# MCG-NJU/MeMOTR

Hardware: AMD Instinct MI355X
Metric: train_frames_per_sec (higher is better)
Workload: dtype f32

## Files before the change

memotr_amd/csrc/clip_ops.hip:

```cpp
#include <hip/hip_runtime.h>
#include <stdint.h>
#include <stdio.h>

#include <atomic>

#include "../../include/clip_ops_hip.h"
#include "assign_core.h"

namespace {

thread_local char g_err[256] = {0};

int fail(int code, const char *msg) {
    snprintf(g_err, sizeof(g_err), "%s", msg);
    return code;
}

int check_launch(const char *what) {
    const hipError_t e = hipGetLastError();
    if (e != hipSuccess) {
        snprintf(g_err, sizeof(g_err), "%s: %s", what, hipGetErrorString(e));
        return (int)e;
    }
    g_err[0] = 0;
// ... 371 lines not shown
    if ((threadIdx.x & 63) == 0) s_w[threadIdx.x >> 6] = a;
    __syncthreads();
    if (threadIdx.x == 0) {
        const f64x4_t t = (s_w[0] + s_w[1]) + (s_w[2] + s_w[3]);
        const f32x4_t r = {(float)t.x, (float)t.y, (float)t.z, (float)t.w};
        *reinterpret_cast<f32x4_t *>(out + c) = r;
    }
}

__device__ __forceinline__ float colsum_ld(const float *x, long i) { return x[i]; }
__device__ __forceinline__ float colsum_ld(const uint16_t *x, long i) {
    return __uint_as_float(((unsigned)x[i]) << 16);
}

template <typename TX>
__global__ __launch_bounds__(256) void colsum_partial_kernel(const TX *__restrict__ x, long rows, int cols,
                                                            int chunk_rows, float *__restrict__ partial) {
    __shared__ double s_part[8][33];
    const int tx = threadIdx.x & 31, ty = threadIdx.x >> 5;
    const int c = blockIdx.x * 32 + tx;
    const long r0 = (long)blockIdx.y * chunk_rows;
    const long r1 = r0 + chunk_rows < rows ? r0 + chunk_rows : rows;
    double a0 = 0., a1 = 0., a2 = 0., a3 = 0.;
    if (c < cols) {
        long r = r0 + ty;
        for (; r + 24 < r1; r += 32) {
            a0 += colsum_ld(x, r * cols + c);
            a1 += colsum_ld(x, (r + 8) * cols + c);
            a2 += colsum_ld(x, (r + 16) * cols + c);
            a3 += colsum_ld(x, (r + 24) * cols + c);
        }
        for (; r < r1; r += 8) a0 += colsum_ld(x, r * cols + c);
    }
    s_part[ty][tx] = (a0 + a1) + (a2 + a3);
    __syncthreads();
    if (ty == 0 && c < cols) {
        double t = s_part[0][tx];
#pragma unroll
        for (int i = 1; i < 8; ++i) t += s_part[i][tx];
        partial[(long)blockIdx.y * cols + c] = (float)t;
    }
}

__device__ __forceinline__ void colsum_st(float *x, long i, float v) { x[i] = v; }

template <typename TX>
__global__ __launch_bounds__(256) void relu_bwd_colsum_partial_kernel(const TX *__restrict__ g, const TX *__restrict__ y,
                                                                     long rows, int cols, int chunk_rows,
                                                                     TX *__restrict__ g2, float *__restrict__ partial) {
    __shared__ double s_part[8][33];
    const int tx = threadIdx.x & 31, ty = threadIdx.x >> 5;
    const int c = blockIdx.x * 32 + tx;
    const long r0 = (long)blockIdx.y * chunk_rows;
    const long r1 = r0 + chunk_rows < rows ? r0 + chunk_rows : rows;
    double a0 = 0., a1 = 0., a2 = 0., a3 = 0.;
    if (c < cols) {
        long r = r0 + ty;
        for (; r + 24 < r1; r += 32) {
            const long i0 = r * cols + c, i1 = (r + 8) * cols + c, i2 = (r + 16) * cols + c, i3 = (r + 24) * cols + c;
            const float v0 = colsum_ld(y, i0) <= 0.f ? 0.f : colsum_ld(g, i0);
            const float v1 = colsum_ld(y, i1) <= 0.f ? 0.f : colsum_ld(g, i1);
            const float v2 = colsum_ld(y, i2) <= 0.f ? 0.f : colsum_ld(g, i2);
            const float v3 = colsum_ld(y, i3) <= 0.f ? 0.f : colsum_ld(g, i3);
            colsum_st(g2, i0, v0); colsum_st(g2, i1, v1); colsum_st(g2, i2, v2); colsum_st(g2, i3, v3);
            a0 += v0; a1 += v1; a2 += v2; a3 += v3;
        }
        for (; r < r1; r += 8) {
            const long i0 = r * cols + c;
            const float v0 = colsum_ld(y, i0) <= 0.f ? 0.f : colsum_ld(g, i0);
            colsum_st(g2, i0, v0);
            a0 += v0;
        }
    }
    s_part[ty][tx] = (a0 + a1) + (a2 + a3);
    __syncthreads();
    if (ty == 0 && c < cols) {
        double t = s_part[0][tx];
#pragma unroll
        for (int i = 1; i < 8; ++i) t += s_part[i][tx];
        partial[(long)blockIdx.y * cols + c] = (float)t;
    }
}

constexpr int kLanes = 16;
constexpr int kRows = 256 / kLanes;
constexpr int kHd = 32;
constexpr int kPitch = 36;

__device__ __forceinline__ void load_row32(const float *p, float *r) {
#pragma unroll
    for (int i = 0; i < 8; ++i) {
        const f32x4_t v = *reinterpret_cast<const f32x4_t *>(p + 4 * i);
        r[4 * i] = v.x; r[4 * i + 1] = v.y; r[4 * i + 2] = v.z; r[4 * i + 3] = v.w;
    }
}

__device__ __forceinline__ float dot32(const float *a, const float *lds_row) {
    float s0 = 0.f, s1 = 0.f;
#pragma unroll
    for (int i = 0; i < 8; ++i) {
        const f32x4_t v = *reinterpret_cast<const f32x4_t *>(lds_row + 4 * i);
        s0 = fmaf(a[4 * i], v.x, s0);
        s1 = fmaf(a[4 * i + 1], v.y, s1);
        s0 = fmaf(a[4 * i + 2], v.z, s0);
        s1 = fmaf(a[4 * i + 3], v.w, s1);
    }
    return s0 + s1;
}

__device__ __forceinline__ float dot32r(const float *a, const float *b) {
    float s0 = 0.f, s1 = 0.f;
#pragma unroll
    for (int i = 0; i < 8; ++i) {
        s0 = fmaf(a[4 * i], b[4 * i], s0);
        s1 = fmaf(a[4 * i + 1], b[4 * i + 1], s1);
        s0 = fmaf(a[4 * i + 2], b[4 * i + 2], s0);
        s1 = fmaf(a[4 * i + 3], b[4 * i + 3], s1);
    }
    return s0 + s1;
}

__device__ __forceinline__ void axpy32(float *acc, float w, const float *lds_row) {
#pragma unroll
    for (int i = 0; i < 8; ++i) {
        const f32x4_t v = *reinterpret_cast<const f32x4_t *>(lds_row + 4 * i);
        acc[4 * i] = fmaf(w, v.x, acc[4 * i]);
        acc[4 * i + 1] = fmaf(w, v.y, acc[4 * i + 1]);
        acc[4 * i + 2] = fmaf(w, v.z, acc[4 * i + 2]);
        acc[4 * i + 3] = fmaf(w, v.w, acc[4 * i + 3]);
    }
}

__device__ __forceinline__ float sum8l(float x) {
#pragma unroll
    for (int o = 1; o < kLanes; o <<= 1) x += __shfl_xor(x, o, 64);
    return x;
}
__device__ __forceinline__ float max8l(float x) {
#pragma unroll
    for (int o = 1; o < kLanes; o <<= 1) x = fmaxf(x, __shfl_xor(x, o, 64));
    return x;
}

__device__ __forceinline__ void stage_rows(float *dst, const float *src, long rs, int L) {
    for (int i = threadIdx.x; i < L * 8; i += blockDim.x) {
        const int r = i >> 3, c = (i & 7) * 4;
        *reinterpret_cast<f32x4_t *>(dst + r * kPitch + c) = *reinterpret_cast<const f32x4_t *>(src + r * rs + c);
    }
}

__global__ __launch_bounds__(256) void mha_fwd_kernel(const float *__restrict__ q, const float *__restrict__ k,
                                                     const float *__restrict__ v, long q_bs, long q_rs, long k_bs,
                                                     long k_rs, long v_bs, long v_rs,
                                                     const uint8_t *__restrict__ key_mask, int H, int L, float scale,
                                                     float *__restrict__ out, float *__restrict__ lse) {
    extern __shared__ __attribute__((aligned(16))) float s_mem[];
    float *Ks = s_mem, *Vs = s_mem + (size_t)L * kPitch;
    const int h = blockIdx.y, b = blockIdx.z;
    stage_rows(Ks, k + b * k_bs + h * kHd, k_rs, L);
    stage_rows(Vs, v + b * v_bs + h * kHd, v_rs, L);
    __syncthreads();
    const int row = blockIdx.x * kRows + threadIdx.x / kLanes, sub = threadIdx.x % kLanes;
    const bool row_ok = row < L;
    const int rowc = row_ok ? row : L - 1;
    float qr[kHd];
    load_row32(q + b * q_bs + rowc * q_rs + h * kHd, qr);
#pragma unroll
    for (int i = 0; i < kHd; ++i) qr[i] *= scale;
    const uint8_t *mk = key_mask ? key_mask + (long)b * L : nullptr;
    float m = -INFINITY, l = 0.f, acc[kHd];
#pragma unroll
    for (int i = 0; i < kHd; ++i) acc[i] = 0.f;
    for (int j = sub; j < L; j += kLanes) {
        if (mk && mk[j]) continue;
        const float s = dot32(qr, Ks + j * kPitch);
        const float m_new = fmaxf(m, s);
        const float corr = expf(m - m_new), p = expf(s - m_new);
        l = l * corr + p;
#pragma unroll
        for (int i = 0; i < kHd; ++i) acc[i] *= corr;
        axpy32(acc, p, Vs + j * kPitch);
        m = m_new;
    }
    const float M = max8l(m);
    const float w = (m == -INFINITY) ? 0.f : expf(m - M);
    const float Lsum = sum8l(l * w);
    const float inv = 1.f / Lsum;
    float *o = out + ((long)b * L + rowc) * (H * kHd) + h * kHd;
#pragma unroll
    for (int i = 0; i < kHd; ++i) {
        const float t = sum8l(acc[i] * w) * inv;
        if (row_ok && (i >> 2) == sub) o[i] = t;
    }
    if (row_ok && sub == 0) lse[((long)b * H + h) * L + row] = M + logf(Lsum);
}

__global__ __launch_bounds__(256) void mha_bwd_q_kernel(const float *__restrict__ q, const float *__restrict__ k,
                                                       const float *__restrict__ v, long q_bs, long q_rs, long k_bs,
                                                       long k_rs, long v_bs, long v_rs,
                                                       const uint8_t *__restrict__ key_mask,
                                                       const float *__restrict__ out, const float *__restrict__ lse,
                                                       const float *__restrict__ go, int H, int L, float scale,
                                                       float *__restrict__ gq, long gq_bs, long gq_rs) {
    extern __shared__ __attribute__((aligned(16))) float s_mem[];
    float *Ks = s_mem, *Vs = s_mem + (size_t)L * kPitch;
    const int h = blockIdx.y, b = blockIdx.z;
    stage_rows(Ks, k + b * k_bs + h * kHd, k_rs, L);
    stage_rows(Vs, v + b * v_bs + h * kHd, v_rs, L);
    __syncthreads();
    const int row = blockIdx.x * kRows + threadIdx.x / kLanes, sub = threadIdx.x % kLanes;
    const bool row_ok = row < L;
    const int rowc = row_ok ? row : L - 1;
    float qr[kHd], gr[kHd], acc[kHd];
    load_row32(q + b * q_bs + rowc * q_rs + h * kHd, qr);
    const long orow = ((long)b * L + rowc) * (H * kHd) + h * kHd;
    load_row32(go + orow, gr);
    float D = 0.f;
    {
        float orr[kHd];
        load_row32(out + orow, orr);
        D = dot32r(gr, orr);
    }
#pragma unroll
    for (int i = 0; i < kHd; ++i) { qr[i] *= scale; acc[i] = 0.f; }
    const float ls = lse[((long)b * H + h) * L + rowc];
    const uint8_t *mk = key_mask ? key_mask + (long)b * L : nullptr;
    for (int j = sub; j < L; j += kLanes) {
        if (mk && mk[j]) continue;
        const float p = expf(dot32(qr, Ks + j * kPitch) - ls);
        const float ds = p * (dot32(gr, Vs + j * kPitch) - D);
        axpy32(acc, ds, Ks + j * kPitch);
    }
    float *g = gq + b * gq_bs + rowc * gq_rs + h * kHd;
#pragma unroll
    for (int i = 0; i < kHd; ++i) {
        const float t = sum8l(acc[i]) * scale;
        if (row_ok && (i >> 2) == sub) g[i] = t;
    }
}

__global__ __launch_bounds__(256) void mha_bwd_kv_kernel(const float *__restrict__ q, const float *__restrict__ k,
                                                        const float *__restrict__ v, long q_bs, long q_rs, long k_bs,
                                                        long k_rs, long v_bs, long v_rs,
                                                        const uint8_t *__restrict__ key_mask,
                                                        const float *__restrict__ out, const float *__restrict__ lse,
                                                        const float *__restrict__ go, int H, int L, float scale,
                                                        float *__restrict__ gk, long gk_bs, long gk_rs,
                                                        float *__restrict__ gv, long gv_bs, long gv_rs) {
    extern __shared__ __attribute__((aligned(16))) float s_mem[];
    float *Qs = s_mem, *Gs = s_mem + (size_t)L * kPitch;
    float *s_lse = Gs + (size_t)L * kPitch, *s_D = s_lse + L;
    const int h = blockIdx.y, b = blockIdx.z;
    stage_rows(Qs, q + b * q_bs + h * kHd, q_rs, L);
    for (int i = threadIdx.x; i < L * 8; i += blockDim.x) {
        f32x4_t *p4 = reinterpret_cast<f32x4_t *>(Qs + (i >> 3) * kPitch + (i & 7) * 4);
        *p4 = *p4 * scale;
    }
    stage_rows(Gs, go + (long)b * L * (H * kHd) + h * kHd, (long)H * kHd, L);
    for (int i = threadIdx.x; i < L; i += blockDim.x) s_lse[i] = lse[((long)b * H + h) * L + i];
    __syncthreads();
    for (int i = threadIdx.x; i < L; i += blockDim.x) {
        const float *o = out + ((long)b * L + i) * (H * kHd) + h * kHd;
        float orr[kHd];
        load_row32(o, orr);
        s_D[i] = dot32(orr, Gs + i * kPitch);
    }
    __syncthreads();
    const int row = blockIdx.x * kRows + threadIdx.x / kLanes, sub = threadIdx.x % kLanes;
    const bool row_ok = row < L;
    const int rowc = row_ok ? row : L - 1;
    const bool dead = key_mask && key_mask[(long)b * L + rowc];
    float kr[kHd], vr[kHd], ak[kHd], av[kHd];
    load_row32(k + b * k_bs + rowc * k_rs + h * kHd, kr);
    load_row32(v + b * v_bs + rowc * v_rs + h * kHd, vr);
#pragma unroll
    for (int i = 0; i < kHd; ++i) { ak[i] = 0.f; av[i] = 0.f; }
    if (!dead) {
        for (int i = sub; i < L; i += kLanes) {
            const float p = expf(dot32(kr, Qs + i * kPitch) - s_lse[i]);
            const float ds = p * (dot32(vr, Gs + i * kPitch) - s_D[i]);
            axpy32(av, p, Gs + i * kPitch);
            axpy32(ak, ds, Qs + i * kPitch);
        }
    }
    float *pk = gk + b * gk_bs + rowc * gk_rs + h * kHd, *pv = gv + b * gv_bs + rowc * gv_rs + h * kHd;
#pragma unroll
    for (int i = 0; i < kHd; ++i) {
        const float tk = sum8l(ak[i]), tv = sum8l(av[i]);
        if (row_ok && (i >> 2) == sub) {
            pk[i] = tk;
            pv[i] = tv;
        }
    }
}

int allow_lds(const void *kernel, size_t lds, std::atomic<unsigned long long> &done) {
    if (lds <= 64 * 1024) return 0;
    int dev = 0;
    (void)hipGetDevice(&dev);
    const unsigned long long bit = 1ull << (dev & 63);
    if (done.load(std::memory_order_acquire) & bit) return 0;
    const hipError_t e = hipFuncSetAttribute(kernel, hipFuncAttributeMaxDynamicSharedMemorySize, 160 * 1024 - 2048);
    if (e != hipSuccess) {
        snprintf(g_err, sizeof(g_err), "hipFuncSetAttribute: %s", hipGetErrorString(e));
        return (int)e;
    }
    done.fetch_or(bit, std::memory_order_release);
    return 0;
}

std::atomic<unsigned long long> g_lds_fwd{0}, g_lds_bq{0}, g_lds_bkv{0};

int mha_check(const void *q, const void *k, const void *v, int B, int H, int L) {
    if (B < 0 || H <= 0 || L < 0) return fail(1, "clipops_mha: bad dimension");
    if (L > CLIPOPS_MHA_MAX_L) return fail(2, "clipops_mha: L exceeds CLIPOPS_MHA_MAX_L");
    if ((long)B * L > 0 && (!q || !k || !v)) return fail(1, "clipops_mha: null pointer");
    return 0;
}

__device__ __forceinline__ float wave_sum64(float x) {
#pragma unroll
    for (int o = 32; o > 0; o >>= 1) x += __shfl_xor(x, o, 64);
    return x;
}

template <bool WITH_Q>
__global__ __launch_bounds__(256) void add_layer_norm_fwd_kernel(const float *__restrict__ x,
                                                                const float *__restrict__ res,
                                                                const float *__restrict__ gamma,
                                                                const float *__restrict__ beta,
                                                                const float *__restrict__ pos, long rows, float eps,
                                                                float *__restrict__ sum, float *__restrict__ y,
                                                                float *__restrict__ q, float *__restrict__ stats) {
    const int lane = threadIdx.x & 63;
    const long row = (long)blockIdx.x * 4 + (threadIdx.x >> 6);
    if (row >= rows) return;
    const long off = row * CLIPOPS_LN_COLS + lane * 4;
    const f32x4_t a = *reinterpret_cast<const f32x4_t *>(x + off);
    const f32x4_t b = *reinterpret_cast<const f32x4_t *>(res + off);
    const f32x4_t s = a + b;
    *reinterpret_cast<f32x4_t *>(sum + off) = s;
    const float mean = wave_sum64((s.x + s.y) + (s.z + s.w)) * (1.f / CLIPOPS_LN_COLS);
    const f32x4_t d = s - mean;
    const float var = wave_sum64((d.x * d.x + d.y * d.y) + (d.z * d.z + d.w * d.w)) * (1.f / CLIPOPS_LN_COLS);
    const float rstd = rsqrtf(var + eps);
    const f32x4_t g = *reinterpret_cast<const f32x4_t *>(gamma + lane * 4);
    const f32x4_t be = *reinterpret_cast<const f32x4_t *>(beta + lane * 4);
    const f32x4_t yv = (d * rstd) * g + be;
    *reinterpret_cast<f32x4_t *>(y + off) = yv;
    if (WITH_Q) *reinterpret_cast<f32x4_t *>(q + off) = yv + *reinterpret_cast<const f32x4_t *>(pos + off);
    if (lane == 0) {
        stats[2 * row] = mean;
        stats[2 * row + 1] = rstd;
    }
}

__global__ __launch_bounds__(256) void add_layer_norm_bwd_kernel(const float *__restrict__ gy,
                                                                const float *__restrict__ sum,
                                                                const float *__restrict__ stats,
                                                                const float *__restrict__ gamma, long rows,
                                                                int chunk_rows, float *__restrict__ gsum,
                                                                float *__restrict__ partial) {
    __shared__ f32x4_t s_acc[4][2][64];
    const int lane = threadIdx.x & 63, wave = threadIdx.x >> 6;
    const f32x4_t gm = *reinterpret_cast<const f32x4_t *>(gamma + lane * 4);
    f32x4_t acc_g = {0.f, 0.f, 0.f, 0.f}, acc_b = {0.f, 0.f, 0.f, 0.f};
    const long r0 = (long)blockIdx.x * chunk_rows;
    const long r1 = r0 + chunk_rows < rows ? r0 + chunk_rows : rows;
    for (long row = r0 + wave; row < r1; row += 4) {
        const long off = row * CLIPOPS_LN_COLS + lane * 4;
        const f32x4_t g = *reinterpret_cast<const f32x4_t *>(gy + off);
        const f32x4_t s = *reinterpret_cast<const f32x4_t *>(sum + off);
        const float mean = stats[2 * row], rstd = stats[2 * row + 1];
        const f32x4_t xh = (s - mean) * rstd;
        const f32x4_t gh = g * gm;
        const float c1 = wave_sum64((gh.x + gh.y) + (gh.z + gh.w)) * (1.f / CLIPOPS_LN_COLS);
        const float c2 = wave_sum64((gh.x * xh.x + gh.y * xh.y) + (gh.z * xh.z + gh.w * xh.w)) * (1.f / CLIPOPS_LN_COLS);
        *reinterpret_cast<f32x4_t *>(gsum + off) = (gh - c1 - xh * c2) * rstd;
        acc_g += g * xh;
        acc_b += g;
    }
    s_acc[wave][0][lane] = acc_g;
    s_acc[wave][1][lane] = acc_b;
    __syncthreads();
    if (wave < 2) {
        const f32x4_t t = (s_acc[0][wave][lane] + s_acc[1][wave][lane]) + (s_acc[2][wave][lane] + s_acc[3][wave][lane]);
        *reinterpret_cast<f32x4_t *>(partial + (long)blockIdx.x * 2 * CLIPOPS_LN_COLS + wave * CLIPOPS_LN_COLS + lane * 4) = t;
    }
}

__global__ __launch_bounds__(256) void add_layer_norm_bwd_fanin_kernel(const float *__restrict__ ga,
                                                                      const float *__restrict__ gb,
                                                                      const float *__restrict__ gc,
                                                                      const float *__restrict__ sum,
// ... 549 lines not shown
    if (!delta || !ref || !out_head || !out_dec) return fail(1, "clipops_refine_boxes_split_fwd_f32: null pointer");
    if (out_head == out_dec) return fail(1, "clipops_refine_boxes_split_fwd_f32: the two outputs alias");
    const bool vec = (((uintptr_t)delta | (uintptr_t)ref | (uintptr_t)out_head | (uintptr_t)out_dec) & 15) == 0;
    if (vec)
        hipLaunchKernelGGL(refine_boxes_split_fwd_kernel<true>, dim3(grid_for(n_rows)), dim3(256), 0,
                           (hipStream_t)stream, delta, ref, n_rows, eps, out_head, out_dec);
    else
        hipLaunchKernelGGL(refine_boxes_split_fwd_kernel<false>, dim3(grid_for(n_rows)), dim3(256), 0,
                           (hipStream_t)stream, delta, ref, n_rows, eps, out_head, out_dec);
    return check_launch("refine_boxes_split_fwd_kernel");
}

int clipops_refine_boxes_bwd_f32(const float *out, const float *ref, const float *grad_out, long n, float eps,
                                 float *grad_delta, float *grad_ref, void *stream) {
    if (n < 0) return fail(1, "clipops_refine_boxes_bwd_f32: negative count");
    if (n == 0) { g_err[0] = 0; return 0; }
    if (!out || !ref || !grad_out || !grad_delta) return fail(1, "clipops_refine_boxes_bwd_f32: null pointer");
    hipLaunchKernelGGL(refine_boxes_bwd_kernel, dim3(grid_for(n)), dim3(256), 0, (hipStream_t)stream, out, ref,
                       grad_out, n, eps, grad_delta, grad_ref);
    return check_launch("refine_boxes_bwd_kernel");
}

int clipops_colsum_f32(const float *x, long rows, int cols, float *out, void *stream) {
    if (rows < 0 || cols < 0) return fail(1, "clipops_colsum_f32: bad dimension");
    if (cols == 0) { g_err[0] = 0; return 0; }
    if (!out || (rows > 0 && !x)) return fail(1, "clipops_colsum_f32: null pointer");
    if (cols % 4 == 0 && rows <= 2048 && (((uintptr_t)x | (uintptr_t)out) & 15) == 0) {
        hipLaunchKernelGGL(colsum_quad_kernel, dim3(cols / 4), dim3(256), 0, (hipStream_t)stream, x, rows, cols, out);
        return check_launch("colsum_quad_kernel");
    }
    hipLaunchKernelGGL(colsum_kernel, dim3((cols + 31) / 32), dim3(256), 0, (hipStream_t)stream, x, rows, cols, out);
    return check_launch("colsum_kernel");
}

int clipops_colsum_partial_f32(const float *x, long rows, int cols, int chunk_rows, float *partial, void *stream) {
    if (rows < 0 || cols < 0 || chunk_rows <= 0) return fail(1, "clipops_colsum_partial_f32: bad dimension");
    if (cols == 0 || rows == 0) { g_err[0] = 0; return 0; }
    if (!x || !partial) return fail(1, "clipops_colsum_partial_f32: null pointer");
    const long chunks = (rows + chunk_rows - 1) / chunk_rows;
    if (chunks > 65535) return fail(1, "clipops_colsum_partial_f32: too many chunks");
    hipLaunchKernelGGL(colsum_partial_kernel<float>, dim3((cols + 31) / 32, (unsigned)chunks), dim3(256), 0,
                       (hipStream_t)stream, x, rows, cols, chunk_rows, partial);
    return check_launch("colsum_partial_kernel");
}

int clipops_colsum_partial_bf16(const uint16_t *x, long rows, int cols, int chunk_rows, float *partial, void *stream) {
    if (rows < 0 || cols < 0 || chunk_rows <= 0) return fail(1, "clipops_colsum_partial_bf16: bad dimension");
    if (cols == 0 || rows == 0) { g_err[0] = 0; return 0; }
    if (!x || !partial) return fail(1, "clipops_colsum_partial_bf16: null pointer");
    const long chunks = (rows + chunk_rows - 1) / chunk_rows;
    if (chunks > 65535) return fail(1, "clipops_colsum_partial_bf16: too many chunks");
    hipLaunchKernelGGL(colsum_partial_kernel<uint16_t>, dim3((cols + 31) / 32, (unsigned)chunks), dim3(256), 0,
                       (hipStream_t)stream, x, rows, cols, chunk_rows, partial);
    return check_launch("colsum_partial_kernel<bf16>");
}

static int relu_bwd_colsum_check(const void *g, const void *y, const void *g2, const void *partial, long rows, int cols,
                                 int chunk_rows, long *chunks) {
    if (rows < 0 || cols < 0 || chunk_rows <= 0) return fail(1, "clipops_relu_bwd_colsum_partial: bad dimension");
    *chunks = (rows + chunk_rows - 1) / chunk_rows;
    if (cols == 0 || rows == 0) return 0;
    if (!g || !y || !g2 || !partial) return fail(1, "clipops_relu_bwd_colsum_partial: null pointer");
    if (*chunks > 65535) return fail(1, "clipops_relu_bwd_colsum_partial: too many chunks");
    return 0;
}

int clipops_relu_bwd_colsum_partial_f32(const float *g, const float *y, long rows, int cols, int chunk_rows, float *g2,
                                        float *partial, void *stream) {
    long chunks = 0;
    if (relu_bwd_colsum_check(g, y, g2, partial, rows, cols, chunk_rows, &chunks)) return 1;
    if (cols == 0 || rows == 0) { g_err[0] = 0; return 0; }
    hipLaunchKernelGGL(relu_bwd_colsum_partial_kernel<float>, dim3((cols + 31) / 32, (unsigned)chunks), dim3(256), 0,
                       (hipStream_t)stream, g, y, rows, cols, chunk_rows, g2, partial);
    return check_launch("relu_bwd_colsum_partial_kernel");
}

int clipops_mha_fwd_f32(const float *q, const float *k, const float *v, long q_bs, long q_rs, long k_bs, long k_rs,
                        long v_bs, long v_rs, const uint8_t *key_mask, int B, int H, int L, float scale, float *out,
                        float *lse, void *stream) {
    int rc = mha_check(q, k, v, B, H, L);
    if (rc) return rc;
    if ((long)B * L == 0) { g_err[0] = 0; return 0; }
    if (!out || !lse) return fail(1, "clipops_mha_fwd_f32: null pointer");
    const size_t lds = (size_t)2 * L * kPitch * sizeof(float);
    if ((rc = allow_lds(reinterpret_cast<const void *>(mha_fwd_kernel), lds, g_lds_fwd))) return rc;
    hipLaunchKernelGGL(mha_fwd_kernel, dim3((L + kRows - 1) / kRows, H, B), dim3(256), lds, (hipStream_t)stream, q, k, v, q_bs,
                       q_rs, k_bs, k_rs, v_bs, v_rs, key_mask, H, L, scale, out, lse);
    return check_launch("mha_fwd_kernel");
}

int clipops_mha_bwd_f32(const float *q, const float *k, const float *v, long q_bs, long q_rs, long k_bs, long k_rs,
                        long v_bs, long v_rs, const uint8_t *key_mask, const float *out, const float *lse,
                        const float *grad_out, int B, int H, int L, float scale, float *grad_q, long gq_bs, long gq_rs,
                        float *grad_k, long gk_bs, long gk_rs, float *grad_v, long gv_bs, long gv_rs, void *stream) {
    int rc = mha_check(q, k, v, B, H, L);
    if (rc) return rc;
    if ((long)B * L == 0) { g_err[0] = 0; return 0; }
    if (!out || !lse || !grad_out || !grad_q || !grad_k || !grad_v) return fail(1, "clipops_mha_bwd_f32: null pointer");
    const size_t lds_q = (size_t)2 * L * kPitch * sizeof(float);
    const size_t lds_kv = lds_q + (size_t)2 * L * sizeof(float);
    if ((rc = allow_lds(reinterpret_cast<const void *>(mha_bwd_q_kernel), lds_q, g_lds_bq))) return rc;
    if ((rc = allow_lds(reinterpret_cast<const void *>(mha_bwd_kv_kernel), lds_kv, g_lds_bkv))) return rc;
    const dim3 grid((L + kRows - 1) / kRows, H, B);
    hipLaunchKernelGGL(mha_bwd_q_kernel, grid, dim3(256), lds_q, (hipStream_t)stream, q, k, v, q_bs, q_rs, k_bs, k_rs,
                       v_bs, v_rs, key_mask, out, lse, grad_out, H, L, scale, grad_q, gq_bs, gq_rs);
    if ((rc = check_launch("mha_bwd_q_kernel"))) return rc;
    hipLaunchKernelGGL(mha_bwd_kv_kernel, grid, dim3(256), lds_kv, (hipStream_t)stream, q, k, v, q_bs, q_rs, k_bs, k_rs,
                       v_bs, v_rs, key_mask, out, lse, grad_out, H, L, scale, grad_k, gk_bs, gk_rs, grad_v, gv_bs, gv_rs);
    return check_launch("mha_bwd_kv_kernel");
}

int clipops_add_layer_norm_fwd_f32(const float *x, const float *res, const float *gamma, const float *beta, long rows,
                                   float eps, float *sum, float *y, float *stats, void *stream) {
    if (rows < 0) return fail(1, "clipops_add_layer_norm_fwd_f32: negative row count");
    if (rows == 0) { g_err[0] = 0; return 0; }
    if (!x || !res || !gamma || !beta || !sum || !y || !stats) return fail(1, "clipops_add_layer_norm_fwd_f32: null pointer");
    hipLaunchKernelGGL(add_layer_norm_fwd_kernel<false>, dim3((unsigned)((rows + 3) / 4)), dim3(256), 0, (hipStream_t)stream,
                       x, res, gamma, beta, nullptr, rows, eps, sum, y, nullptr, stats);
    return check_launch("add_layer_norm_fwd_kernel");
}

int clipops_add_layer_norm_pos_fwd_f32(const float *x, const float *res, const float *gamma, const float *beta,
                                       const float *pos, long rows, float eps, float *sum, float *y, float *q,
                                       float *stats, void *stream) {
    if (rows < 0) return fail(1, "clipops_add_layer_norm_pos_fwd_f32: negative row count");
    if (rows == 0) { g_err[0] = 0; return 0; }
    if (!x || !res || !gamma || !beta || !pos || !sum || !y || !q || !stats)
        return fail(1, "clipops_add_layer_norm_pos_fwd_f32: null pointer");
    hipLaunchKernelGGL(add_layer_norm_fwd_kernel<true>, dim3((unsigned)((rows + 3) / 4)), dim3(256), 0, (hipStream_t)stream,
                       x, res, gamma, beta, pos, rows, eps, sum, y, q, stats);
    return check_launch("add_layer_norm_fwd_kernel<pos>");
}

int clipops_add_layer_norm_bwd_f32(const float *grad_y, const float *sum, const float *stats, const float *gamma,
                                   long rows, int chunk_rows, float *grad_sum, float *partial, void *stream) {
    if (rows < 0 || chunk_rows <= 0) return fail(1, "clipops_add_layer_norm_bwd_f32: bad dimension");
    if (rows == 0) { g_err[0] = 0; return 0; }
    if (!grad_y || !sum || !stats || !gamma || !grad_sum || !partial)
        return fail(1, "clipops_add_layer_norm_bwd_f32: null pointer");
    hipLaunchKernelGGL(add_layer_norm_bwd_kernel, dim3((unsigned)((rows + chunk_rows - 1) / chunk_rows)), dim3(256), 0,
                       (hipStream_t)stream, grad_y, sum, stats, gamma, rows, chunk_rows, grad_sum, partial);
    return check_launch("add_layer_norm_bwd_kernel");
}

int clipops_add_layer_norm_fanin_bwd_f32(const float *g0, const float *g1, const float *g2, const float *sum,
                                         const float *stats, const float *gamma, long rows, int chunk_rows,
                                         float *grad_sum, float *partial, float *colsum_partial, void *stream) {
    if (rows < 0 || chunk_rows <= 0) return fail(1, "clipops_add_layer_norm_fanin_bwd_f32: bad dimension");
    if (rows == 0) { g_err[0] = 0; return 0; }
    const float *g[3] = {nullptr, nullptr, nullptr};
    int n = 0;
    if (g0) g[n++] = g0;
    if (g1) g[n++] = g1;
    if (g2) g[n++] = g2;
    if (n == 0) return fail(1, "clipops_add_layer_norm_fanin_bwd_f32: no gradient input");
    if (!sum || !stats || !gamma || !grad_sum || !partial || !colsum_partial)
        return fail(1, "clipops_add_layer_norm_fanin_bwd_f32: null pointer");
    hipLaunchKernelGGL(add_layer_norm_bwd_fanin_kernel, dim3((unsigned)((rows + chunk_rows - 1) / chunk_rows)), dim3(256), 0,
                       (hipStream_t)stream, g[0], g[1], g[2], sum, stats, gamma, rows, chunk_rows, grad_sum, partial,
                       colsum_partial);
    return check_launch("add_layer_norm_bwd_fanin_kernel");
}

int clipops_assign_f32(const float *cost, long stride_problem, long stride_row, long stride_col, int n_problems,
                       int n_rows, int n_cols, int32_t *row_ind, int32_t *col_ind, int32_t *status, void *stream) {
    if (n_problems < 0 || n_rows < 0 || n_cols < 0) return fail(1, "clipops_assign_f32: bad dimension");
    if (n_problems == 0 || n_rows == 0 || n_cols == 0) { g_err[0] = 0; return 0; }
    if (!cost || !row_ind || !col_ind) return fail(1, "clipops_assign_f32: null pointer");
    const int nr = n_rows < n_cols ? n_rows : n_cols, nc = n_rows < n_cols ? n_cols : n_rows;
    if (nc > CLIPOPS_ASSIGN_MAX_DIM) return fail(2, "clipops_assign_f32: problem exceeds CLIPOPS_ASSIGN_MAX_DIM");
    const size_t lds = (assign::work_bytes(nr, nc) + 15) & ~(size_t)15;
    if (lds > 64 * 1024) {
        static std::atomic<size_t> allowed{0};
        if (lds > 160 * 1024) return fail(2, "clipops_assign_f32: problem does not fit the LDS of a CU");
        if (lds > allowed.load()) {
            if (hipFuncSetAttribute(reinterpret_cast<const void *>(assign_kernel),
                                    hipFuncAttributeMaxDynamicSharedMemorySize, 160 * 1024) != hipSuccess) {
                (void)hipGetLastError();
                return fail(3, "clipops_assign_f32: hipFuncSetAttribute(MaxDynamicSharedMemorySize) failed");
            }
            allowed.store(160 * 1024);
        }
    }
    hipLaunchKernelGGL(assign_kernel, dim3(n_problems), dim3(64), lds, (hipStream_t)stream, cost, stride_problem,
                       stride_row, stride_col, n_rows, n_cols, row_ind, col_ind, status);
    return check_launch("assign_kernel");
}

static int shift_relu_check(const void *x, const void *shift, long planes, int C, long HW, const char *who) {
    if (planes < 0 || C <= 0 || HW < 0) return fail(1, who);
    if (planes && HW && (!x || !shift)) return fail(1, who);
    return 0;
// ... 63 lines not shown
```

Baseline: 42.34.

## Rewrite MHA forward/backward on f32 MFMA tiles with split-K waves

Replaces the scalar per-lane attention kernels, which staged all of K/V in LDS, with 32x32 tile kernels built on the f32 32x32x2 MFMA instruction. Each of four waves handles a strided slice of keys and keeps its own online-softmax state, and the slices are merged through shared memory. The two backward kernels become one launch whose blocks split into dQ tiles and dK/dV tiles. This removes the large dynamic LDS requirement and the scalar FMA cost, in exchange for direct global loads that are not reused across the block, extra reductions through shared memory, and the backward recomputing D per tile.

Result: no change. 42.51 (median of 5 runs) (+0.4%).

```diff
diff --git a/memotr_amd/csrc/clip_ops.hip b/memotr_amd/csrc/clip_ops.hip
--- a/memotr_amd/csrc/clip_ops.hip
+++ b/memotr_amd/csrc/clip_ops.hip
@@ -477,70 +477,94 @@
     }
 }
 
-constexpr int kLanes = 16;
-constexpr int kRows = 256 / kLanes;
 constexpr int kHd = 32;
-constexpr int kPitch = 36;
-
-__device__ __forceinline__ void load_row32(const float *p, float *r) {
-#pragma unroll
-    for (int i = 0; i < 8; ++i) {
-        const f32x4_t v = *reinterpret_cast<const f32x4_t *>(p + 4 * i);
-        r[4 * i] = v.x; r[4 * i + 1] = v.y; r[4 * i + 2] = v.z; r[4 * i + 3] = v.w;
-    }
-}
-
-__device__ __forceinline__ float dot32(const float *a, const float *lds_row) {
-    float s0 = 0.f, s1 = 0.f;
-#pragma unroll
-    for (int i = 0; i < 8; ++i) {
-        const f32x4_t v = *reinterpret_cast<const f32x4_t *>(lds_row + 4 * i);
-        s0 = fmaf(a[4 * i], v.x, s0);
-        s1 = fmaf(a[4 * i + 1], v.y, s1);
-        s0 = fmaf(a[4 * i + 2], v.z, s0);
-        s1 = fmaf(a[4 * i + 3], v.w, s1);
-    }
-    return s0 + s1;
-}
-
-__device__ __forceinline__ float dot32r(const float *a, const float *b) {
-    float s0 = 0.f, s1 = 0.f;
-#pragma unroll
-    for (int i = 0; i < 8; ++i) {
-        s0 = fmaf(a[4 * i], b[4 * i], s0);
-        s1 = fmaf(a[4 * i + 1], b[4 * i + 1], s1);
-        s0 = fmaf(a[4 * i + 2], b[4 * i + 2], s0);
-        s1 = fmaf(a[4 * i + 3], b[4 * i + 3], s1);
-    }
-    return s0 + s1;
-}
-
-__device__ __forceinline__ void axpy32(float *acc, float w, const float *lds_row) {
-#pragma unroll
-    for (int i = 0; i < 8; ++i) {
-        const f32x4_t v = *reinterpret_cast<const f32x4_t *>(lds_row + 4 * i);
-        acc[4 * i] = fmaf(w, v.x, acc[4 * i]);
-        acc[4 * i + 1] = fmaf(w, v.y, acc[4 * i + 1]);
-        acc[4 * i + 2] = fmaf(w, v.z, acc[4 * i + 2]);
-        acc[4 * i + 3] = fmaf(w, v.w, acc[4 * i + 3]);
-    }
-}
-
-__device__ __forceinline__ float sum8l(float x) {
-#pragma unroll
-    for (int o = 1; o < kLanes; o <<= 1) x += __shfl_xor(x, o, 64);
-    return x;
-}
-__device__ __forceinline__ float max8l(float x) {
-#pragma unroll
-    for (int o = 1; o < kLanes; o <<= 1) x = fmaxf(x, __shfl_xor(x, o, 64));
-    return x;
-}
-
-__device__ __forceinline__ void stage_rows(float *dst, const float *src, long rs, int L) {
-    for (int i = threadIdx.x; i < L * 8; i += blockDim.x) {
-        const int r = i >> 3, c = (i & 7) * 4;
-        *reinterpret_cast<f32x4_t *>(dst + r * kPitch + c) = *reinterpret_cast<const f32x4_t *>(src + r * rs + c);
+constexpr int kTile = 32;
+typedef float mha_f32x16 __attribute__((ext_vector_type(16)));
+
+struct MhaRows { f32x4_t c[4]; };
+
+__device__ __forceinline__ int mha_row(int r, int hf) { return (r & 3) + 8 * (r >> 2) + 4 * hf; }
+
+__device__ __forceinline__ mha_f32x16 mha_zero() {
+    return mha_f32x16{0.f, 0.f, 0.f, 0.f, 0.f, 0.f, 0.f, 0.f, 0.f, 0.f, 0.f, 0.f, 0.f, 0.f, 0.f, 0.f};
+}
+
+__device__ __forceinline__ MhaRows mha_load_rows(const float *base, long rs, int row, int n, int hf) {
+    MhaRows o;
+    const float *p = base + (long)(row < n ? row : 0) * rs + 4 * hf;
+#pragma unroll
+    for (int c = 0; c < 4; ++c)
+        o.c[c] = row < n ? *reinterpret_cast<const f32x4_t *>(p + 8 * c) : f32x4_t{0.f, 0.f, 0.f, 0.f};
+    return o;
+}
+
+__device__ __forceinline__ void mha_load_cols(float (&o)[16], const float *base, long rs, int row0, int n, int hf,
+                                              int col, float mul) {
+#pragma unroll
+    for (int r = 0; r < 16; ++r) {
+        const int row = row0 + mha_row(r, hf);
+        o[r] = row < n ? base[(long)row * rs + col] * mul : 0.f;
+    }
+}
+
+__device__ __forceinline__ void mha_keep_rows(float (&o)[16], unsigned keep) {
+#pragma unroll
+    for (int r = 0; r < 16; ++r) o[r] = (keep >> r & 1u) ? o[r] : 0.f;
+}
+
+__device__ __forceinline__ mha_f32x16 mha_rows_dot(const MhaRows &a, const MhaRows &b) {
+    mha_f32x16 acc = mha_zero();
+#pragma unroll
+    for (int c = 0; c < 4; ++c) {
+        acc = __builtin_amdgcn_mfma_f32_32x32x2f32(a.c[c].x, b.c[c].x, acc, 0, 0, 0);
+        acc = __builtin_amdgcn_mfma_f32_32x32x2f32(a.c[c].y, b.c[c].y, acc, 0, 0, 0);
+        acc = __builtin_amdgcn_mfma_f32_32x32x2f32(a.c[c].z, b.c[c].z, acc, 0, 0, 0);
+        acc = __builtin_amdgcn_mfma_f32_32x32x2f32(a.c[c].w, b.c[c].w, acc, 0, 0, 0);
+    }
+    return acc;
+}
+
+__device__ __forceinline__ mha_f32x16 mha_cols_acc(const float (&x)[16], const mha_f32x16 &w, mha_f32x16 acc) {
+#pragma unroll
+    for (int r = 0; r < 16; ++r) acc = __builtin_amdgcn_mfma_f32_32x32x2f32(x[r], w[r], acc, 0, 0, 0);
+    return acc;
+}
+
+__device__ __forceinline__ float mha_row_dot_diag(const MhaRows &o, const MhaRows &g, int hf, int col) {
+    const mha_f32x16 x = mha_rows_dot(o, g);
+    float d = 0.f;
+#pragma unroll
+    for (int r = 0; r < 16; ++r) d = (mha_row(r, hf) == col) ? x[r] : d;
+    const float other = __shfl_xor(d, 32, 64);
+    return ((col >> 2 & 1) == hf) ? d : other;
+}
+
+__device__ __forceinline__ unsigned mha_live_keys(const uint8_t *mk, int j0, int hf, int L) {
+    const int j = j0 + (int)(threadIdx.x & 31);
+    const unsigned block = (unsigned)__ballot(j < L && !(mk && mk[j]));
+    unsigned live = 0;
+#pragma unroll
+    for (int r = 0; r < 16; ++r) live |= (block >> mha_row(r, hf) & 1u) << r;
+    return live;
+}
+
+__device__ __forceinline__ void mha_reduce_store(const mha_f32x16 &acc, float (*s_acc)[16][64], float (*s_o)[kTile + 1],
+                                                 float mul, float *dst, long rs, int row0, int n,
+                                                 const uint8_t *zero_rows) {
+    const int lane = threadIdx.x & 63, wave = threadIdx.x >> 6, hf = lane >> 5, col = lane & 31;
+#pragma unroll
+    for (int r = 0; r < 16; ++r) s_acc[wave][r][lane] = acc[r];
+    __syncthreads();
+#pragma unroll
+    for (int rr = 0; rr < 4; ++rr) {
+        const int r = wave * 4 + rr;
+        s_o[col][mha_row(r, hf)] = ((s_acc[0][r][lane] + s_acc[1][r][lane]) + (s_acc[2][r][lane] + s_acc[3][r][lane])) * mul;
+    }
+    __syncthreads();
+#pragma unroll
+    for (int rr = 0; rr < 4; ++rr) {
+        const int t = (int)(threadIdx.x >> 5) + 8 * rr, row = row0 + t;
+        if (row < n) dst[(long)row * rs + col] = (zero_rows && zero_rows[row]) ? 0.f : s_o[t][col];
     }
 }
 
@@ -549,162 +573,156 @@
                                                      long k_rs, long v_bs, long v_rs,
                                                      const uint8_t *__restrict__ key_mask, int H, int L, float scale,
                                                      float *__restrict__ out, float *__restrict__ lse) {
-    extern __shared__ __attribute__((aligned(16))) float s_mem[];
-    float *Ks = s_mem, *Vs = s_mem + (size_t)L * kPitch;
+    __shared__ float s_acc[4][16][64];
+    __shared__ float s_m[4][kTile], s_l[4][kTile];
+    __shared__ float s_o[kTile][kTile + 1];
+    const int lane = threadIdx.x & 63, wave = threadIdx.x >> 6, hf = lane >> 5, col = lane & 31;
+    const int h = blockIdx.y, b = blockIdx.z, i0 = blockIdx.x * kTile;
+    const float *kb = k + b * k_bs + h * kHd, *vb = v + b * v_bs + h * kHd;
+    MhaRows qs = mha_load_rows(q + b * q_bs + h * kHd, q_rs, i0 + col, L, hf);
+#pragma unroll
+    for (int c = 0; c < 4; ++c) qs.c[c] = qs.c[c] * scale;
+    const uint8_t *mk = key_mask ? key_mask + (long)b * L : nullptr;
+    float m = -INFINITY, l = 0.f;
+    mha_f32x16 acc = mha_zero();
+    for (int j0 = wave * kTile; j0 < L; j0 += 4 * kTile) {
+        const unsigned live = mha_live_keys(mk, j0, hf, L);
+        const MhaRows kr = mha_load_rows(kb, k_rs, j0 + col, L, hf);
+        float vc[16];
+        mha_load_cols(vc, vb, v_rs, j0, L, hf, col, 1.f);
+        mha_keep_rows(vc, live);
+        mha_f32x16 s = mha_rows_dot(kr, qs);
+        float bm = -INFINITY;
+#pragma unroll
+        for (int r = 0; r < 16; ++r) {
+            s[r] = (live >> r & 1u) ? s[r] : -INFINITY;
+            bm = fmaxf(bm, s[r]);
+        }
+        bm = fmaxf(bm, __shfl_xor(bm, 32, 64));
+        const float m_new = fmaxf(m, bm);
+        const float m_ref = (m_new == -INFINITY) ? 0.f : m_new;
+        const float corr = expf(m - m_ref);
+        float ps = 0.f;
+#pragma unroll
+        for (int r = 0; r < 16; ++r) {
+            s[r] = (live >> r & 1u) ? expf(s[r] - m_ref) : 0.f;
+            ps += s[r];
+        }
+        ps += __shfl_xor(ps, 32, 64);
+        l = l * corr + ps;
+#pragma unroll
+        for (int r = 0; r < 16; ++r) acc[r] *= corr;
+        acc = mha_cols_acc(vc, s, acc);
+        m = m_new;
+    }
+#pragma unroll
+    for (int r = 0; r < 16; ++r) s_acc[wave][r][lane] = acc[r];
+    if (hf == 0) {
+        s_m[wave][col] = m;
+        s_l[wave][col] = l;
+    }
+    __syncthreads();
+    const float M = fmaxf(fmaxf(s_m[0][col], s_m[1][col]), fmaxf(s_m[2][col], s_m[3][col]));
+    float w[4];
+#pragma unroll
+    for (int u = 0; u < 4; ++u) w[u] = (s_m[u][col] == -INFINITY) ? 0.f : expf(s_m[u][col] - M);
+    const float Lsum = (s_l[0][col] * w[0] + s_l[1][col] * w[1]) + (s_l[2][col] * w[2] + s_l[3][col] * w[3]);
+    const float inv = 1.f / Lsum;
+#pragma unroll
+    for (int rr = 0; rr < 4; ++rr) {
+        const int r = wave * 4 + rr;
+        s_o[col][mha_row(r, hf)] = ((s_acc[0][r][lane] * w[0] + s_acc[1][r][lane] * w[1]) +
+                                    (s_acc[2][r][lane] * w[2] + s_acc[3][r][lane] * w[3])) * inv;
+    }
+    __syncthreads();
+#pragma unroll
+    for (int rr = 0; rr < 4; ++rr) {
+        const int t = (int)(threadIdx.x >> 5) + 8 * rr, row = i0 + t;
+        if (row < L) out[((long)b * L + row) * (H * kHd) + h * kHd + col] = s_o[t][col];
+    }
+    if (wave == 0 && hf == 0 && i0 + col < L) lse[((long)b * H + h) * L + i0 + col] = M + logf(Lsum);
+}
+
+__global__ __launch_bounds__(256) void mha_bwd_kernel(const float *__restrict__ q, const float *__restrict__ k,
+                                                     const float *__restrict__ v, long q_bs, long q_rs, long k_bs,
+                                                     long k_rs, long v_bs, long v_rs,
+                                                     const uint8_t *__restrict__ key_mask,
+                                                     const float *__restrict__ out, const float *__restrict__ lse,
+                                                     const float *__restrict__ go, int H, int L, float scale,
+                                                     float *__restrict__ gq, long gq_bs, long gq_rs,
+                                                     float *__restrict__ gk, long gk_bs, long gk_rs,
+                                                     float *__restrict__ gv, long gv_bs, long gv_rs, int n_tiles) {
+    __shared__ float s_acc[4][16][64];
+    __shared__ float s_o[kTile][kTile + 1];
+    const int lane = threadIdx.x & 63, wave = threadIdx.x >> 6, hf = lane >> 5, col = lane & 31;
     const int h = blockIdx.y, b = blockIdx.z;
-    stage_rows(Ks, k + b * k_bs + h * kHd, k_rs, L);
-    stage_rows(Vs, v + b * v_bs + h * kHd, v_rs, L);
-    __syncthreads();
-    const int row = blockIdx.x * kRows + threadIdx.x / kLanes, sub = threadIdx.x % kLanes;
-    const bool row_ok = row < L;
-    const int rowc = row_ok ? row : L - 1;
-    float qr[kHd];
-    load_row32(q + b * q_bs + rowc * q_rs + h * kHd, qr);
-#pragma unroll
-    for (int i = 0; i < kHd; ++i) qr[i] *= scale;
+    const long HE = (long)H * kHd;
+    const float *qb = q + b * q_bs + h * kHd, *kb = k + b * k_bs + h * kHd, *vb = v + b * v_bs + h * kHd;
+    const float *ob = out + (long)b * L * HE + h * kHd, *gb = go + (long)b * L * HE + h * kHd;
+    const float *lb = lse + ((long)b * H + h) * L;
     const uint8_t *mk = key_mask ? key_mask + (long)b * L : nullptr;
-    float m = -INFINITY, l = 0.f, acc[kHd];
-#pragma unroll
-    for (int i = 0; i < kHd; ++i) acc[i] = 0.f;
-    for (int j = sub; j < L; j += kLanes) {
-        if (mk && mk[j]) continue;
-        const float s = dot32(qr, Ks + j * kPitch);
-        const float m_new = fmaxf(m, s);
-        const float corr = expf(m - m_new), p = expf(s - m_new);
-        l = l * corr + p;
-#pragma unroll
-        for (int i = 0; i < kHd; ++i) acc[i] *= corr;
-        axpy32(acc, p, Vs + j * kPitch);
-        m = m_new;
-    }
-    const float M = max8l(m);
-    const float w = (m == -INFINITY) ? 0.f : expf(m - M);
-    const float Lsum = sum8l(l * w);
-    const float inv = 1.f / Lsum;
-    float *o = out + ((long)b * L + rowc) * (H * kHd) + h * kHd;
-#pragma unroll
-    for (int i = 0; i < kHd; ++i) {
-        const float t = sum8l(acc[i] * w) * inv;
-        if (row_ok && (i >> 2) == sub) o[i] = t;
-    }
-    if (row_ok && sub == 0) lse[((long)b * H + h) * L + row] = M + logf(Lsum);
-}
-
-__global__ __launch_bounds__(256) void mha_bwd_q_kernel(const float *__restrict__ q, const float *__restrict__ k,
-                                                       const float *__restrict__ v, long q_bs, long q_rs, long k_bs,
-                                                       long k_rs, long v_bs, long v_rs,
-                                                       const uint8_t *__restrict__ key_mask,
-                                                       const float *__restrict__ out, const float *__restrict__ lse,
-                                                       const float *__restrict__ go, int H, int L, float scale,
-                                                       float *__restrict__ gq, long gq_bs, long gq_rs) {
-    extern __shared__ __attribute__((aligned(16))) float s_mem[];
-    float *Ks = s_mem, *Vs = s_mem + (size_t)L * kPitch;
-    const int h = blockIdx.y, b = blockIdx.z;
-    stage_rows(Ks, k + b * k_bs + h * kHd, k_rs, L);
-    stage_rows(Vs, v + b * v_bs + h * kHd, v_rs, L);
-    __syncthreads();
-    const int row = blockIdx.x * kRows + threadIdx.x / kLanes, sub = threadIdx.x % kLanes;
-    const bool row_ok = row < L;
-    const int rowc = row_ok ? row : L - 1;
-    float qr[kHd], gr[kHd], acc[kHd];
-    load_row32(q + b * q_bs + rowc * q_rs + h * kHd, qr);
-    const long orow = ((long)b * L + rowc) * (H * kHd) + h * kHd;
-    load_row32(go + orow, gr);
-    float D = 0.f;
-    {
-        float orr[kHd];
-        load_row32(out + orow, orr);
-        D = dot32r(gr, orr);
-    }
-#pragma unroll
-    for (int i = 0; i < kHd; ++i) { qr[i] *= scale; acc[i] = 0.f; }
-    const float ls = lse[((long)b * H + h) * L + rowc];
-    const uint8_t *mk = key_mask ? key_mask + (long)b * L : nullptr;
-    for (int j = sub; j < L; j += kLanes) {
-        if (mk && mk[j]) continue;
-        const float p = expf(dot32(qr, Ks + j * kPitch) - ls);
-        const float ds = p * (dot32(gr, Vs + j * kPitch) - D);
-        axpy32(acc, ds, Ks + j * kPitch);
-    }
-    float *g = gq + b * gq_bs + rowc * gq_rs + h * kHd;
-#pragma unroll
-    for (int i = 0; i < kHd; ++i) {
-        const float t = sum8l(acc[i]) * scale;
-        if (row_ok && (i >> 2) == sub) g[i] = t;
-    }
-}
-
-__global__ __launch_bounds__(256) void mha_bwd_kv_kernel(const float *__restrict__ q, const float *__restrict__ k,
-                                                        const float *__restrict__ v, long q_bs, long q_rs, long k_bs,
-                                                        long k_rs, long v_bs, long v_rs,
-                                                        const uint8_t *__restrict__ key_mask,
-                                                        const float *__restrict__ out, const float *__restrict__ lse,
-                                                        const float *__restrict__ go, int H, int L, float scale,
-                                                        float *__restrict__ gk, long gk_bs, long gk_rs,
-                                                        float *__restrict__ gv, long gv_bs, long gv_rs) {
-    extern __shared__ __attribute__((aligned(16))) float s_mem[];
-    float *Qs = s_mem, *Gs = s_mem + (size_t)L * kPitch;
-    float *s_lse = Gs + (size_t)L * kPitch, *s_D = s_lse + L;
-    const int h = blockIdx.y, b = blockIdx.z;
-    stage_rows(Qs, q + b * q_bs + h * kHd, q_rs, L);
-    for (int i = threadIdx.x; i < L * 8; i += blockDim.x) {
-        f32x4_t *p4 = reinterpret_cast<f32x4_t *>(Qs + (i >> 3) * kPitch + (i & 7) * 4);
-        *p4 = *p4 * scale;
-    }
-    stage_rows(Gs, go + (long)b * L * (H * kHd) + h * kHd, (long)H * kHd, L);
-    for (int i = threadIdx.x; i < L; i += blockDim.x) s_lse[i] = lse[((long)b * H + h) * L + i];
-    __syncthreads();
-    for (int i = threadIdx.x; i < L; i += blockDim.x) {
-        const float *o = out + ((long)b * L + i) * (H * kHd) + h * kHd;
-        float orr[kHd];
-        load_row32(o, orr);
-        s_D[i] = dot32(orr, Gs + i * kPitch);
-    }
-    __syncthreads();
-    const int row = blockIdx.x * kRows + threadIdx.x / kLanes, sub = threadIdx.x % kLanes;
-    const bool row_ok = row < L;
-    const int rowc = row_ok ? row : L - 1;
-    const bool dead = key_mask && key_mask[(long)b * L + rowc];
-    float kr[kHd], vr[kHd], ak[kHd], av[kHd];
-    load_row32(k + b * k_bs + rowc * k_rs + h * kHd, kr);
-    load_row32(v + b * v_bs + rowc * v_rs + h * kHd, vr);
-#pragma unroll
-    for (int i = 0; i < kHd; ++i) { ak[i] = 0.f; av[i] = 0.f; }
-    if (!dead) {
-        for (int i = sub; i < L; i += kLanes) {
-            const float p = expf(dot32(kr, Qs + i * kPitch) - s_lse[i]);
-            const float ds = p * (dot32(vr, Gs + i * kPitch) - s_D[i]);
-            axpy32(av, p, Gs + i * kPitch);
-            axpy32(ak, ds, Qs + i * kPitch);
-        }
-    }
-    float *pk = gk + b * gk_bs + rowc * gk_rs + h * kHd, *pv = gv + b * gv_bs + rowc * gv_rs + h * kHd;
-#pragma unroll
-    for (int i = 0; i < kHd; ++i) {
-        const float tk = sum8l(ak[i]), tv = sum8l(av[i]);
-        if (row_ok && (i >> 2) == sub) {
-            pk[i] = tk;
-            pv[i] = tv;
-        }
-    }
-}
-
-int allow_lds(const void *kernel, size_t lds, std::atomic<unsigned long long> &done) {
-    if (lds <= 64 * 1024) return 0;
-    int dev = 0;
-    (void)hipGetDevice(&dev);
-    const unsigned long long bit = 1ull << (dev & 63);
-    if (done.load(std::memory_order_acquire) & bit) return 0;
-    const hipError_t e = hipFuncSetAttribute(kernel, hipFuncAttributeMaxDynamicSharedMemorySize, 160 * 1024 - 2048);
-    if (e != hipSuccess) {
-        snprintf(g_err, sizeof(g_err), "hipFuncSetAttribute: %s", hipGetErrorString(e));
-        return (int)e;
-    }
-    done.fetch_or(bit, std::memory_order_release);
-    return 0;
-}
-
-std::atomic<unsigned long long> g_lds_fwd{0}, g_lds_bq{0}, g_lds_bkv{0};
+    if ((int)blockIdx.x < n_tiles) {
+        const int i0 = blockIdx.x * kTile, i = i0 + col;
+        MhaRows qs = mha_load_rows(qb, q_rs, i, L, hf);
+#pragma unroll
+        for (int c = 0; c < 4; ++c) qs.c[c] = qs.c[c] * scale;
+        const MhaRows gr = mha_load_rows(gb, HE, i, L, hf);
+        const float D = mha_row_dot_diag(mha_load_rows(ob, HE, i, L, hf), gr, hf, col);
+        const float ls = lb[i < L ? i : L - 1];
+        mha_f32x16 acc = mha_zero();
+        for (int j0 = wave * kTile; j0 < L; j0 += 4 * kTile) {
+            const unsigned live = mha_live_keys(mk, j0, hf, L);
+            const MhaRows kr = mha_load_rows(kb, k_rs, j0 + col, L, hf);
+            const MhaRows vr = mha_load_rows(vb, v_rs, j0 + col, L, hf);
+            float kc[16];
+            mha_load_cols(kc, kb, k_rs, j0, L, hf, col, 1.f);
+            mha_keep_rows(kc, live);
+            const mha_f32x16 s = mha_rows_dot(kr, qs);
+            const mha_f32x16 dp = mha_rows_dot(vr, gr);
+            mha_f32x16 ds;
+#pragma unroll
+            for (int r = 0; r < 16; ++r) ds[r] = (live >> r & 1u) ? expf(s[r] - ls) * (dp[r] - D) : 0.f;
+            acc = mha_cols_acc(kc, ds, acc);
+        }
+        mha_reduce_store(acc, s_acc, s_o, scale, gq + b * gq_bs + h * kHd, gq_rs, i0, L, nullptr);
+    } else {
+        const int j0 = ((int)blockIdx.x - n_tiles) * kTile, j = j0 + col;
+        const MhaRows kr = mha_load_rows(kb, k_rs, j, L, hf);
+        const MhaRows vr = mha_load_rows(vb, v_rs, j, L, hf);
+        const bool key_live = j < L && !(mk && mk[j]);
+        mha_f32x16 ak = mha_zero(), av = mha_zero();
+        for (int i0 = wave * kTile; i0 < L; i0 += 4 * kTile) {
+            const int i = i0 + col;
+            MhaRows qs = mha_load_rows(qb, q_rs, i, L, hf);
+#pragma unroll
+            for (int c = 0; c < 4; ++c) qs.c[c] = qs.c[c] * scale;
+            const MhaRows gr = mha_load_rows(gb, HE, i, L, hf);
+            const float D_l = mha_row_dot_diag(mha_load_rows(ob, HE, i, L, hf), gr, hf, col);
+            const float ls_l = lb[i < L ? i : L - 1];
+            unsigned rows = 0;
+#pragma unroll
+            for (int r = 0; r < 16; ++r) rows |= (i0 + mha_row(r, hf) < L ? 1u : 0u) << r;
+            float qc[16], gc[16];
+            mha_load_cols(qc, qb, q_rs, i0, L, hf, col, scale);
+            mha_load_cols(gc, gb, HE, i0, L, hf, col, 1.f);
+            const mha_f32x16 s = mha_rows_dot(qs, kr);
+            const mha_f32x16 dp = mha_rows_dot(gr, vr);
+            mha_f32x16 p, ds;
+#pragma unroll
+            for (int r = 0; r < 16; ++r) {
+                const int src = mha_row(r, hf);
+                const float D = __shfl(D_l, src, 64), ls = __shfl(ls_l, src, 64);
+                const bool on = key_live && (rows >> r & 1u);
+                p[r] = on ? expf(s[r] - ls) : 0.f;
+                ds[r] = on ? p[r] * (dp[r] - D) : 0.f;
+            }
+            av = mha_cols_acc(gc, p, av);
+            ak = mha_cols_acc(qc, ds, ak);
+        }
+        mha_reduce_store(ak, s_acc, s_o, 1.f, gk + b * gk_bs + h * kHd, gk_rs, j0, L, mk);
+        mha_reduce_store(av, s_acc, s_o, 1.f, gv + b * gv_bs + h * kHd, gv_rs, j0, L, mk);
+    }
+}
 
 int mha_check(const void *q, const void *k, const void *v, int B, int H, int L) {
     if (B < 0 || H <= 0 || L < 0) return fail(1, "clipops_mha: bad dimension");
@@ -1420,9 +1438,7 @@
     if (rc) return rc;
     if ((long)B * L == 0) { g_err[0] = 0; return 0; }
     if (!out || !lse) return fail(1, "clipops_mha_fwd_f32: null pointer");
-    const size_t lds = (size_t)2 * L * kPitch * sizeof(float);
-    if ((rc = allow_lds(reinterpret_cast<const void *>(mha_fwd_kernel), lds, g_lds_fwd))) return rc;
-    hipLaunchKernelGGL(mha_fwd_kernel, dim3((L + kRows - 1) / kRows, H, B), dim3(256), lds, (hipStream_t)stream, q, k, v, q_bs,
+    hipLaunchKernelGGL(mha_fwd_kernel, dim3((L + kTile - 1) / kTile, H, B), dim3(256), 0, (hipStream_t)stream, q, k, v, q_bs,
                        q_rs, k_bs, k_rs, v_bs, v_rs, key_mask, H, L, scale, out, lse);
     return check_launch("mha_fwd_kernel");
 }
@@ -1435,17 +1451,11 @@
     if (rc) return rc;
     if ((long)B * L == 0) { g_err[0] = 0; return 0; }
     if (!out || !lse || !grad_out || !grad_q || !grad_k || !grad_v) return fail(1, "clipops_mha_bwd_f32: null pointer");
-    const size_t lds_q = (size_t)2 * L * kPitch * sizeof(float);
-    const size_t lds_kv = lds_q + (size_t)2 * L * sizeof(float);
-    if ((rc = allow_lds(reinterpret_cast<const void *>(mha_bwd_q_kernel), lds_q, g_lds_bq))) return rc;
-    if ((rc = allow_lds(reinterpret_cast<const void *>(mha_bwd_kv_kernel), lds_kv, g_lds_bkv))) return rc;
-    const dim3 grid((L + kRows - 1) / kRows, H, B);
-    hipLaunchKernelGGL(mha_bwd_q_kernel, grid, dim3(256), lds_q, (hipStream_t)stream, q, k, v, q_bs, q_rs, k_bs, k_rs,
-                       v_bs, v_rs, key_mask, out, lse, grad_out, H, L, scale, grad_q, gq_bs, gq_rs);
-    if ((rc = check_launch("mha_bwd_q_kernel"))) return rc;
-    hipLaunchKernelGGL(mha_bwd_kv_kernel, grid, dim3(256), lds_kv, (hipStream_t)stream, q, k, v, q_bs, q_rs, k_bs, k_rs,
-                       v_bs, v_rs, key_mask, out, lse, grad_out, H, L, scale, grad_k, gk_bs, gk_rs, grad_v, gv_bs, gv_rs);
-    return check_launch("mha_bwd_kv_kernel");
+    const int n_tiles = (L + kTile - 1) / kTile;
+    hipLaunchKernelGGL(mha_bwd_kernel, dim3(2 * n_tiles, H, B), dim3(256), 0, (hipStream_t)stream, q, k, v, q_bs, q_rs, k_bs,
+                       k_rs, v_bs, v_rs, key_mask, out, lse, grad_out, H, L, scale, grad_q, gq_bs, gq_rs, grad_k, gk_bs, gk_rs,
+                       grad_v, gv_bs, gv_rs, n_tiles);
+    return check_launch("mha_bwd_kernel");
 }
 
 int clipops_add_layer_norm_fwd_f32(const float *x, const float *res, const float *gamma, const float *beta, long rows,
```
